# explosion/spacy-ray

Hardware: AMD Instinct MI355X
Metric: words/sec (whole node) en_core CNN tagger+parser+NER train (higher is better)
Workload: dtype bf16; 1 GPU; global_batch=1000015, seq_len=20, parallelism=dp1

## Files before the change

spacy_ray_amd/ops/api.py:

```python
from __future__ import annotations

import os
from typing import Optional

import torch

from . import torch_ref as ref

_HIP = None
_HIP_TRIED = False

FIXED_SCALE = 16777216.0


def deterministic() -> bool:
    return os.environ.get("SRX_DETERMINISTIC") == "1"


def hip_ext():
    global _HIP, _HIP_TRIED
    if not _HIP_TRIED:
        _HIP_TRIED = True
        try:
            from spacy_ray_amd import _srx_hip
# ... 717 lines not shown
    def forward(ctx, x, grad_buf):
        ctx.grad_buf = grad_buf
        ctx.dtype = x.dtype
        return x.new_zeros(())

    @staticmethod
    def backward(ctx, g):
        return ctx.grad_buf.to(ctx.dtype) * g, None


def inject_grad(x: torch.Tensor, grad_buf: torch.Tensor) -> torch.Tensor:
    return _InjectGrad.apply(x, grad_buf)


def parser_scatter_entries(entries, dPre32) -> None:
    if not entries:
        return
    hip = hip_ext()
    device = dPre32.device
    nF = entries[0][0].shape[1]
    HP = dPre32.shape[-1]
    feats_all = torch.cat([f for f, _ in entries], dim=0)
    dS_all = torch.cat([d for _, d in entries], dim=0).contiguous()
    SS = feats_all.shape[0]
    slot = torch.arange(nF, device=device)
    dest = (feats_all * nF + slot).reshape(-1).int()
    src = torch.arange(SS, device=device, dtype=torch.int32).repeat_interleave(nF)
    order = torch.argsort(dest)
    hip.seg_scatter_add(dest[order].contiguous(), src[order].contiguous(),
                        dS_all, dPre32.view(-1, HP))


class _MWELayer(torch.autograd.Function):

    @staticmethod
    def forward(ctx, X, weight, bias, g, b, starts, ends, dropmask, eps):
        Y, Mout, which, mu, rstd = hip_ext().mwe_layer_fwd(
            X.contiguous(), weight, bias, g, b, starts, ends, dropmask, eps
        )
        ctx.save_for_backward(X, weight, g, which, Mout, mu, rstd, starts, ends,
                              *( [dropmask] if dropmask is not None else [] ))
        ctx.has_mask = dropmask is not None
        return Y

    @staticmethod
    def backward(ctx, dY):
        if ctx.has_mask:
            X, weight, g, which, Mout, mu, rstd, starts, ends, dropmask = ctx.saved_tensors
        else:
            X, weight, g, which, Mout, mu, rstd, starts, ends = ctx.saved_tensors
            dropmask = None
        hip = hip_ext()
        dY = dY.contiguous()
        dPre, dX, dg32, db32, dbias32 = hip.mwe_bwd_fused(
            dY, dropmask, Mout, g, mu, rstd, which, weight, starts, ends)
        X3 = hip.seq2col_fwd(X, starts, ends)
        dW = mm_dw_chunked(dPre, X3)
        return (dX, dW, dbias32.to(dY.dtype), dg32.to(dY.dtype),
                db32.to(dY.dtype), None, None, None, None)


def mwe_layer(X, weight, bias, g, b, starts, ends, dropmask=None, eps: float = 1e-5):
    return _MWELayer.apply(X, weight, bias, g, b, starts, ends, dropmask, eps)


def mwe_layer_available(X: torch.Tensor, width: int, pieces: int) -> bool:
    return (
        X.is_cuda
        and X.dtype == torch.bfloat16
        and pieces == 3
        and width in (96, 128)
        and X.shape[0] % 64 == 0
        and hip_ext() is not None
    )


class _MixerLayer(torch.autograd.Function):

    @staticmethod
    def forward(ctx, E, weight, bias, g, b, dropmask, eps):
        E = E.contiguous()
        Y, Mout, which, mu, rstd = hip_ext().mixer_fwd(
            E, weight, bias, g, b, dropmask, eps)
        ctx.save_for_backward(E, weight, g, which, Mout, mu, rstd,
                              *([dropmask] if dropmask is not None else []))
        ctx.has_mask = dropmask is not None
        return Y

    @staticmethod
    def backward(ctx, dY):
        if ctx.has_mask:
            E, weight, g, which, Mout, mu, rstd, dropmask = ctx.saved_tensors
        else:
            E, weight, g, which, Mout, mu, rstd = ctx.saved_tensors
            dropmask = None
        dY = dY.contiguous()
        dPre, dE, dg32, db32, dbias32 = hip_ext().mixer_bwd_fused(
            dY, dropmask, Mout, g, mu, rstd, which, weight)
        dW = mm_dw_chunked(dPre, E)
        return (dE, dW, dbias32.to(dY.dtype), dg32.to(dY.dtype),
                db32.to(dY.dtype), None, None)


def mixer_layer(E, weight, bias, g, b, dropmask=None, eps: float = 1e-5):
    return _MixerLayer.apply(E, weight, bias, g, b, dropmask, eps)


def _mixer_composed() -> bool:
    mode = os.environ.get("SRX_MIXER", "")
    if mode not in ("", "composed"):
        raise ValueError(f"SRX_MIXER={mode!r}: expected 'composed' or unset")
    return mode == "composed"
# ... 271 lines not shown
```

spacy_ray_amd/ops/kernels/srx_ext.hip:

```cpp
#include <torch/extension.h>
#include <ATen/cuda/CUDAContext.h>

#include <mutex>
#include <unordered_map>
#include <utility>
#include <vector>

#include "srx_common.hip.h"
#include "srx_elementwise.hip.h"
#include "srx_embed_parser.hip.h"
#include "srx_softmax_reduce.hip.h"
#include "srx_mwe.hip.h"
#include "srx_mixer.hip.h"
#include "srx_staticvec.hip.h"
#include "srx_floret.hip.h"
#include "srx_vecloss.hip.h"
#include "srx_activations.hip.h"
#include "srx_attn.hip.h"

namespace {

constexpr int kBlock = 256;

inline int grid_for(long total, int per_thread = 1) {
  long blocks = (total + (long)kBlock * per_thread - 1) / ((long)kBlock * per_thread);
  return (int)std::min<long>(blocks, 16384);
}

inline void check_dev(const at::Tensor& t) {
  TORCH_CHECK(t.is_cuda(), "expected a GPU tensor");
  TORCH_CHECK(t.is_contiguous(), "expected contiguous");
}

#define DISPATCH_F(dtype, ...)                                        \
  if ((dtype) == at::kFloat) {                                        \
    using scalar_t = float;                                           \
    constexpr int kVec = 4;                                           \
    __VA_ARGS__;                                                      \
  } else if ((dtype) == at::kBFloat16) {                              \
    using scalar_t = bf16_t;                                          \
    constexpr int kVec = 8;                                           \
    __VA_ARGS__;                                                      \
  } else {                                                            \
    TORCH_CHECK(false, "unsupported dtype (need f32 or bf16)");       \
  }

at::Tensor seq2col_fwd(at::Tensor X, at::Tensor starts, at::Tensor ends) {
  check_dev(X);
  long nT = X.size(0);
  int W = (int)X.size(1);
  auto Y = at::empty({nT, 3L * W}, X.options());
  if (nT == 0) return Y;
  auto stream = at::cuda::getCurrentCUDAStream();
  DISPATCH_F(X.scalar_type(), {
    const int V = (W % kVec == 0) ? kVec : 1;
    long total = nT * 3L * (W / V);
    if (V == kVec)
      hipLaunchKernelGGL((seq2col_fwd_kernel<scalar_t, kVec>), dim3(grid_for(total)),
                         dim3(kBlock), 0, stream,
                         (const scalar_t*)X.data_ptr(), (scalar_t*)Y.data_ptr(),
                         starts.data_ptr<uint8_t>(), ends.data_ptr<uint8_t>(), nT, W);
    else
      hipLaunchKernelGGL((seq2col_fwd_kernel<scalar_t, 1>), dim3(grid_for(nT * 3L * W)),
                         dim3(kBlock), 0, stream,
                         (const scalar_t*)X.data_ptr(), (scalar_t*)Y.data_ptr(),
                         starts.data_ptr<uint8_t>(), ends.data_ptr<uint8_t>(), nT, W);
// ... 1058 lines not shown
  dim3 grid((unsigned)((T + C::MT - 1) / C::MT));
  hipLaunchKernelGGL((mwe_bwd_dx_kernel<W>), grid, dim3(C::NT), lds_bytes, stream,
                     (const bf16_t*)dPre.data_ptr(), (const bf16_t*)WT.data_ptr(),
                     starts.data_ptr<uint8_t>(), ends.data_ptr<uint8_t>(),
                     (const bf16_t*)dY.data_ptr(), (bf16_t*)dX.data_ptr(), T);
}

at::Tensor mwe_bwd_dx(at::Tensor dPre, at::Tensor weight, at::Tensor starts,
                      at::Tensor ends, at::Tensor dY) {
  check_dev(dPre);
  check_dev(dY);
  TORCH_CHECK(weight.is_cuda(), "expected a GPU tensor");
  TORCH_CHECK(dPre.scalar_type() == at::kBFloat16 &&
                  weight.scalar_type() == at::kBFloat16 &&
                  dY.scalar_type() == at::kBFloat16,
              "mwe_bwd_dx is bf16-only");
  TORCH_CHECK(dPre.dim() == 2 && dY.dim() == 2 && weight.dim() == 2,
              "mwe_bwd_dx expects 2-d tensors");
  long T = dY.size(0);
  int W = (int)dY.size(1);
  TORCH_CHECK(W == 96 || W == 128, "mwe_bwd_dx supports W in {96,128}");
  TORCH_CHECK(T % 64 == 0, "mwe_bwd_dx needs T % 64 == 0 (TokenBatch pads)");
  TORCH_CHECK(dPre.size(0) == T && dPre.size(1) == 3 * W, "dPre must be [T,3W]");
  TORCH_CHECK(weight.size(0) == 3 * W && weight.size(1) == 3 * W,
              "weight must be [3W,3W]");
  TORCH_CHECK(starts.numel() == T && ends.numel() == T,
              "starts/ends must have T entries");
  auto dX = at::empty_like(dY);
  if (T == 0) return dX;
  auto WT = weight.t().contiguous();
  auto stream = at::cuda::getCurrentCUDAStream();
  if (W == 96)
    launch_mwe_bwd_dx<96>(dPre, WT, starts, ends, dY, dX, T, stream);
  else
    launch_mwe_bwd_dx<128>(dPre, WT, starts, ends, dY, dX, T, stream);
  return dX;
}

at::Tensor mwe_fold_partials(at::Tensor part, int ncols, hipStream_t stream) {
  long n = part.size(0);
  const int R = 64;
  do {
    long nb = (n + R - 1) / R;
    auto out = at::empty({nb, (long)ncols}, part.options());
    hipLaunchKernelGGL(mwe_colsum_kernel, dim3((unsigned)nb, (ncols + 63) / 64),
                       dim3(64), 0, stream, part.data_ptr<float>(),
                       out.data_ptr<float>(), n, R, ncols);
    part = out;
    n = nb;
  } while (n > 1);
  return part.view({(long)ncols});
}

template <int W>
void launch_mwe_bwd_fused(const at::Tensor& dY,
                          const c10::optional<at::Tensor>& dropmask,
                          const at::Tensor& Mout, const at::Tensor& g,
                          const at::Tensor& mu, const at::Tensor& rstd,
                          const at::Tensor& which, const at::Tensor& WT,
                          const at::Tensor& starts, const at::Tensor& ends,
                          at::Tensor& dPre, at::Tensor& dX, at::Tensor& partials,
                          long T, hipStream_t stream) {
  using C = MweCfg<W, true>;
  size_t lds_bytes = (size_t)(C::A_ELEMS + C::B_ELEMS) * sizeof(bf16_t);
  static bool attr_set = false;
  if (!attr_set) {
    (void)hipFuncSetAttribute((const void*)mwe_bwd_fused_kernel<W>,
                              hipFuncAttributeMaxDynamicSharedMemorySize,
                              (int)lds_bytes);
    attr_set = true;
  }
  dim3 grid((unsigned)((T + C::MT - 1) / C::MT));
  hipLaunchKernelGGL((mwe_bwd_fused_kernel<W>), grid, dim3(C::NT), lds_bytes,
                     stream, (const bf16_t*)dY.data_ptr(),
                     dropmask ? (const bf16_t*)dropmask->data_ptr() : nullptr,
                     (const bf16_t*)Mout.data_ptr(), (const bf16_t*)g.data_ptr(),
                     mu.data_ptr<float>(), rstd.data_ptr<float>(),
                     which.data_ptr<uint8_t>(), (const bf16_t*)WT.data_ptr(),
                     starts.data_ptr<uint8_t>(), ends.data_ptr<uint8_t>(),
                     (bf16_t*)dPre.data_ptr(), (bf16_t*)dX.data_ptr(),
                     partials.data_ptr<float>(), T);
}

std::vector<at::Tensor> mwe_bwd_fused(at::Tensor dY,
                                      c10::optional<at::Tensor> dropmask,
                                      at::Tensor Mout, at::Tensor g,
                                      at::Tensor mu, at::Tensor rstd,
                                      at::Tensor which, at::Tensor weight,
                                      at::Tensor starts, at::Tensor ends) {
  check_dev(dY);
  check_dev(Mout);
  check_dev(g);
  check_dev(mu);
  check_dev(rstd);
  check_dev(which);
  check_dev(starts);
  check_dev(ends);
  TORCH_CHECK(weight.is_cuda(), "expected a GPU tensor");
  TORCH_CHECK(dY.scalar_type() == at::kBFloat16 &&
                  Mout.scalar_type() == at::kBFloat16 &&
                  g.scalar_type() == at::kBFloat16 &&
                  weight.scalar_type() == at::kBFloat16,
              "mwe_bwd_fused is bf16-only");
  TORCH_CHECK(dY.dim() == 2 && weight.dim() == 2,
              "mwe_bwd_fused expects 2-d tensors");
  long T = dY.size(0);
  int W = (int)dY.size(1);
  TORCH_CHECK(W == 96 || W == 128, "mwe_bwd_fused supports W in {96,128}");
  TORCH_CHECK(T % 64 == 0, "mwe_bwd_fused needs T % 64 == 0 (TokenBatch pads)");
  TORCH_CHECK(weight.size(0) == 3 * W && weight.size(1) == 3 * W,
              "weight must be [3W,3W]");
  TORCH_CHECK(starts.numel() == T && ends.numel() == T,
              "starts/ends must have T entries");
  TORCH_CHECK(starts.scalar_type() == at::kByte && ends.scalar_type() == at::kByte,
              "starts/ends must be uint8");
  TORCH_CHECK(Mout.dim() == 2 && Mout.size(0) == T && Mout.size(1) == W,
              "Mout must be [T,W]");
  TORCH_CHECK(which.scalar_type() == at::kByte && which.dim() == 2 &&
                  which.size(0) == T && which.size(1) == W,
              "which must be uint8 [T,W]");
  TORCH_CHECK(mu.scalar_type() == at::kFloat && rstd.scalar_type() == at::kFloat &&
                  mu.numel() == T && rstd.numel() == T,
              "mu/rstd must be fp32 with T entries");
  TORCH_CHECK(g.numel() == W, "g must have W entries");
  if (dropmask) {
    check_dev(*dropmask);
    TORCH_CHECK(dropmask->scalar_type() == at::kBFloat16 && dropmask->dim() == 2 &&
                    dropmask->size(0) == T && dropmask->size(1) == W,
                "dropmask must be bf16 [T,W]");
  }
  auto dPre = at::empty({T, 3L * W}, dY.options());
  auto dX = at::empty_like(dY);
  auto f32 = dY.options().dtype(at::kFloat);
  if (T == 0) {
    return {dPre, dX, at::zeros({W}, f32), at::zeros({W}, f32),
            at::zeros({3L * W}, f32)};
  }
  auto WT = weight.t().contiguous();
  auto stream = at::cuda::getCurrentCUDAStream();
  const int ncols = 5 * W;
  long n = (T + 127) / 128;
  auto part = at::empty({n, (long)ncols}, f32);
  if (W == 96)
    launch_mwe_bwd_fused<96>(dY, dropmask, Mout, g, mu, rstd, which, WT, starts,
                             ends, dPre, dX, part, T, stream);
  else
    launch_mwe_bwd_fused<128>(dY, dropmask, Mout, g, mu, rstd, which, WT, starts,
                              ends, dPre, dX, part, T, stream);
  auto sums = mwe_fold_partials(part, ncols, stream);
  return {dPre, dX, sums.narrow(0, 0, W), sums.narrow(0, W, W),
          sums.narrow(0, 2L * W, 3L * W)};
}

void mixer_check_shape(const char* name, long T, int W, int NS) {
  TORCH_CHECK(W == 96 || W == 128, name, " supports W in {96,128}");
  TORCH_CHECK(NS == 4 || NS == 5, name, " supports 4 or 5 input blocks of width W");
  TORCH_CHECK(T % 64 == 0, name, " needs T % 64 == 0 (TokenBatch pads)");
}

void mixer_check_mask(const c10::optional<at::Tensor>& dropmask, long T, int W) {
  if (!dropmask) return;
  check_dev(*dropmask);
  TORCH_CHECK(dropmask->scalar_type() == at::kBFloat16 && dropmask->dim() == 2 &&
                  dropmask->size(0) == T && dropmask->size(1) == W,
              "dropmask must be bf16 [T,W]");
}

template <int W, int NS>
void launch_mixer_fwd(const at::Tensor& E, const at::Tensor& Wm,
                      const at::Tensor& bias, const at::Tensor& g,
                      const at::Tensor& b,
                      const c10::optional<at::Tensor>& dropmask, at::Tensor& Y,
                      at::Tensor& Mout, at::Tensor& which, at::Tensor& mu,
                      at::Tensor& rstd, long T, double eps, hipStream_t stream) {
  using C = MixCfg<W, NS, false>;
  size_t lds_bytes = MixFwdLds<W, NS>::BYTES;
  static bool attr_set = false;
  if (!attr_set) {
    (void)hipFuncSetAttribute((const void*)mixer_fwd_kernel<W, NS>,
                              hipFuncAttributeMaxDynamicSharedMemorySize,
                              (int)lds_bytes);
    attr_set = true;
  }
  dim3 grid((unsigned)((T + C::MT - 1) / C::MT));
  hipLaunchKernelGGL((mixer_fwd_kernel<W, NS>), grid, dim3(C::NT), lds_bytes,
                     stream, (const bf16_t*)E.data_ptr(), (const bf16_t*)Wm.data_ptr(),
                     (const bf16_t*)bias.data_ptr(), (const bf16_t*)g.data_ptr(),
                     (const bf16_t*)b.data_ptr(),
                     dropmask ? (const bf16_t*)dropmask->data_ptr() : nullptr,
                     (bf16_t*)Y.data_ptr(), (bf16_t*)Mout.data_ptr(),
                     which.data_ptr<uint8_t>(), mu.data_ptr<float>(),
                     rstd.data_ptr<float>(), T, (float)eps);
}

std::vector<at::Tensor> mixer_fwd(at::Tensor E, at::Tensor Wm, at::Tensor bias,
                                  at::Tensor g, at::Tensor b,
                                  c10::optional<at::Tensor> dropmask, double eps) {
  check_dev(E);
  check_dev(Wm);
  check_dev(bias);
  check_dev(g);
  check_dev(b);
  TORCH_CHECK(E.scalar_type() == at::kBFloat16 &&
                  Wm.scalar_type() == at::kBFloat16 &&
// ... 442 lines not shown

std::vector<at::Tensor> srx_gpu_arceager(
    at::Tensor pre, at::Tensor off, at::Tensor lens, at::Tensor gh,
    at::Tensor gl, at::Tensor kids_off, at::Tensor kids, at::Tensor lowerB,
    at::Tensor upperW, at::Tensor upperB, int64_t total, int64_t n_labels,
    bool train, bool fuse_ce);
std::vector<at::Tensor> srx_gpu_biluo(
    at::Tensor pre, at::Tensor off, at::Tensor lens, at::Tensor gold,
    at::Tensor lowerB, at::Tensor upperW, at::Tensor upperB, int64_t total,
    int64_t n_types, bool train, bool fuse_ce);

PYBIND11_MODULE(TORCH_EXTENSION_NAME, m) {
  m.def("seq2col_fwd", &seq2col_fwd);
  m.def("seq2col_bwd", &seq2col_bwd, py::arg("dY"), py::arg("starts"),
        py::arg("ends"), py::arg("residual") = py::none());
  m.def("mwe_bwd_stage1", &mwe_bwd_stage1, py::arg("dY"), py::arg("dropmask"),
        py::arg("Mout"), py::arg("g"), py::arg("mu"), py::arg("rstd"),
        py::arg("which"), py::arg("deterministic") = false);
  m.def("maxout_fwd", &maxout_fwd);
  m.def("maxout_bwd", &maxout_bwd);
  m.def("layernorm_fwd", &layernorm_fwd);
  m.def("layernorm_bwd", &layernorm_bwd, py::arg("dY"), py::arg("X"),
        py::arg("g"), py::arg("mu"), py::arg("rstd"),
        py::arg("deterministic") = false);
  m.def("hashembed_fwd", &hashembed_fwd, py::arg("table"), py::arg("ids"),
        py::arg("seed"), py::arg("out") = py::none(), py::arg("col_off") = 0);
  m.def("hashembed_bwd", &hashembed_bwd);
  m.def("multi_hashembed_fwd", &multi_hashembed_fwd, py::arg("ids4"),
        py::arg("tables"), py::arg("seeds"), py::arg("X"), py::arg("col_off") = 0);
  m.def("hashembed_bwd_merged", &hashembed_bwd_merged, py::arg("order"),
        py::arg("rows"), py::arg("dY"), py::arg("dT32"));
  m.def("parser_step_fwd", &parser_step_fwd);
  m.def("parser_step_bwd", &parser_step_bwd);
  m.def("parser_step_bwd_into", &parser_step_bwd_into);
  m.def("action_select", &action_select);
  m.def("seg_scatter_add", &seg_scatter_add);
  m.def("adam_step", &adam_step);
  m.def("dropout_mask", &dropout_mask);
  m.def("act_fwd", &act_fwd);
  m.def("attn_softmax_fwd", &attn_softmax_fwd);
  m.def("attn_fused_fwd", &attn_fused_fwd);
  m.def("attn_fused_bwd", &attn_fused_bwd);
  m.def("attn_softmax_bwd", &attn_softmax_bwd);
  m.def("act_bwd", &act_bwd);
  m.def("softmax_ce", &softmax_ce);
  m.def("reduce_ragged", &reduce_ragged);
  m.def("reduce_ragged_bwd", &reduce_ragged_bwd);
  m.def("reduce_max_bwd", &reduce_max_bwd);
  m.def("mwe_layer_fwd", &mwe_layer_fwd);
  m.def("mwe_bwd_dx", &mwe_bwd_dx, py::arg("dPre"), py::arg("weight"),
        py::arg("starts"), py::arg("ends"), py::arg("dY"));
  m.def("mwe_bwd_fused", &mwe_bwd_fused, py::arg("dY"), py::arg("dropmask"),
        py::arg("Mout"), py::arg("g"), py::arg("mu"), py::arg("rstd"),
        py::arg("which"), py::arg("weight"), py::arg("starts"), py::arg("ends"));
  m.def("mixer_fwd", &mixer_fwd, py::arg("E"), py::arg("weight"), py::arg("bias"),
        py::arg("g"), py::arg("b"), py::arg("dropmask"), py::arg("eps"));
  m.def("mixer_bwd_fused", &mixer_bwd_fused, py::arg("dY"), py::arg("dropmask"),
        py::arg("Mout"), py::arg("g"), py::arg("mu"), py::arg("rstd"),
        py::arg("which"), py::arg("weight"));
  m.def("static_vectors_fwd", &static_vectors_fwd, py::arg("table"),
        py::arg("rows"), py::arg("W"), py::arg("Y"), py::arg("col_off") = 0);
  m.def("static_vectors_bwd_dw", &static_vectors_bwd_dw, py::arg("table"),
        py::arg("rows"), py::arg("dX"), py::arg("col_off"), py::arg("nO"),
        py::arg("max_groups") = 0, py::arg("nM") = 0);
  m.def("floret_words_mean", &floret_words_mean, py::arg("table"),
        py::arg("offsets"), py::arg("idx"), py::arg("out"));
  m.def("vectors_loss", &vectors_loss, py::arg("pred"), py::arg("table"),
        py::arg("rows"), py::arg("row_loss"), py::arg("dpred"), py::arg("l2"),
        py::arg("scale"));
  m.def("fused_step", &fusedstep::fused_step);
  m.def("fused_entries_take", &fusedstep::fused_entries_take);
  m.def("transition_ce", &transition_ce, py::arg("scores"), py::arg("gold"),
        py::arg("valid"), py::arg("deterministic") = false);
  m.attr("FIXED_SCALE") = 16777216.0;
  m.def("dpre_scatter", &dpre_scatter);
  m.def("dpre_scatter_docmajor", &dpre_scatter_docmajor);
  m.def("run_transition_loop", &srx_run_transition_loop,
        py::call_guard<py::gil_scoped_release>());
  m.def("gpu_arceager", &srx_gpu_arceager, py::arg("pre"), py::arg("off"),
        py::arg("lens"), py::arg("gh"), py::arg("gl"), py::arg("kids_off"),
        py::arg("kids"), py::arg("lowerB"), py::arg("upperW"),
        py::arg("upperB"), py::arg("total"), py::arg("n_labels"),
        py::arg("train"), py::arg("fuse_ce") = false);
  m.def("gpu_biluo", &srx_gpu_biluo, py::arg("pre"), py::arg("off"),
        py::arg("lens"), py::arg("gold"), py::arg("lowerB"), py::arg("upperW"),
        py::arg("upperB"), py::arg("total"), py::arg("n_types"),
        py::arg("train"), py::arg("fuse_ce") = false);
  m.attr("GPU_STATE_MAXLEN") = 128;
}
```

spacy_ray_amd/ops/kernels/srx_mwe.hip.h:

```cpp
#pragma once
#include "srx_common.hip.h"

typedef __attribute__((__vector_size__(8 * sizeof(short)))) short srx_bf16x8;
typedef __attribute__((__vector_size__(16 * sizeof(float)))) float srx_f32x16;

template <int W_, bool BWD_>
struct MweCfg {
  static constexpr int W = W_;
  static constexpr bool BWD = BWD_;
  static constexpr int NW = W / 32;
  static constexpr int MT = 128;
  static constexpr int NT = 64 * 2 * NW;
  static constexpr int KA = BWD ? 3 * W : W;
  static constexpr int AP = KA + 8;
  static constexpr int KC = BWD ? 96 : 32;
  static constexpr int BP = KC + 8;
  static constexpr int NBR = BWD ? W : 3 * W;
  static constexpr int LDB = 3 * W;
  static constexpr int NP = BWD ? 1 : 3;
  static constexpr int CPS = KA / KC;
  static constexpr int NC = 3 * CPS;
  static constexpr int PF = NBR * (KC / 8) / NT;
  static constexpr int A_ROWS = MT + 2;
  static constexpr int A_ELEMS = A_ROWS * AP;
// ... 392 lines not shown
  const long nwaves = ((long)gridDim.x * blockDim.x) / SRX_WAVE;
  const int ncols = (W + SRX_WAVE - 1) / SRX_WAVE;
  float dg_loc[4], db_loc[4], dbias_loc[4 * 3];
  for (int c = 0; c < ncols; c++) { dg_loc[c] = 0.f; db_loc[c] = 0.f; }
  for (int k = 0; k < ncols * 3; k++) dbias_loc[k] = 0.f;
  for (long n = wave; n < N; n += nwaves) {
    const T* dyrow = dY + n * (long)W;
    const T* mrow = Mout + n * (long)W;
    const T* maskrow = dropmask ? dropmask + n * (long)W : nullptr;
    float m = mu[n], r = rstd[n];
    float s1 = 0.f, s2 = 0.f;
    float dl[4], xh[4];
    for (int c = 0; c < ncols; c++) {
      int w = lane + c * SRX_WAVE;
      if (w >= W) { dl[c] = 0.f; xh[c] = 0.f; continue; }
      float d = Elem<T>::ld(dyrow + w);
      if (maskrow) d *= Elem<T>::ld(maskrow + w);
      float xhat = (Elem<T>::ld(mrow + w) - m) * r;
      float dxhat = d * Elem<T>::ld(g + w);
      dl[c] = d;
      xh[c] = xhat;
      s1 += dxhat;
      s2 += dxhat * xhat;
      dg_loc[c] += d * xhat;
      db_loc[c] += d;
    }
    s1 = wave_reduce_sum(s1) / W;
    s2 = wave_reduce_sum(s2) / W;
    T* out = dPre + n * (long)(3 * W);
    const uint8_t* wrow = which + n * (long)W;
    for (int c = 0; c < ncols; c++) {
      int w = lane + c * SRX_WAVE;
      if (w >= W) continue;
      float dxhat = dl[c] * Elem<T>::ld(g + w);
      float dM = r * (dxhat - s1 - xh[c] * s2);
      int p = wrow[w];
      for (int q = 0; q < 3; q++)
        Elem<T>::st(out + q * W + w, q == p ? dM : 0.f);
      dbias_loc[c * 3 + p] += dM;
    }
  }
  for (int c = 0; c < ncols; c++) {
    int w = lane + c * SRX_WAVE;
    if (w >= W) continue;
    if (dg_loc[c] != 0.f) srx_atomic_add<DET>(dg32, w, dg_loc[c]);
    if (db_loc[c] != 0.f) srx_atomic_add<DET>(db32, w, db_loc[c]);
    for (int q = 0; q < 3; q++)
      if (dbias_loc[c * 3 + q] != 0.f)
        srx_atomic_add<DET>(dbias32, (long)q * W + w, dbias_loc[c * 3 + q]);
  }
}


template <int W, int NT, int AP, int HALO>
__device__ __forceinline__ void mwe_stage1_tile(
    const bf16_t* __restrict__ dY, const bf16_t* __restrict__ dropmask,
    const bf16_t* __restrict__ Mout, const bf16_t* __restrict__ g,
    const float* __restrict__ mu, const float* __restrict__ rstd,
    const uint8_t* __restrict__ which, long T, long t0, int tid, bf16_t* ldsA,
    float (&dg_out)[8], float (&db_out)[8], float (&dbias_out)[3][8]) {
  constexpr int MT = 128, A_ROWS = MT + 2 * HALO;
  constexpr int Q = W / 8;
  constexpr int RG = NT / 16;
  constexpr int NPASS = (A_ROWS + RG - 1) / RG;
  const int q = tid & 15, rg = tid >> 4;
  const bool qv = q < Q;
  float gv[8];
#pragma unroll
  for (int j = 0; j < 8; j++) gv[j] = 0.f;
  if (qv) ElemV<bf16_t, 8>::ld(g + q * 8, gv);

  srx_u32x4_t rdy[NPASS], rmk[NPASS], rmo[NPASS];
  uint2 rwh[NPASS];
  float rmu[NPASS], rrs[NPASS];
#pragma unroll
  for (int ps = 0; ps < NPASS; ps++) {
    const int i = ps * RG + rg;
    const long t = t0 - HALO + i;
    rdy[ps] = srx_u32x4_t{0u, 0u, 0u, 0u};
    rmk[ps] = srx_u32x4_t{0u, 0u, 0u, 0u};
    rmo[ps] = srx_u32x4_t{0u, 0u, 0u, 0u};
    rwh[ps] = make_uint2(0u, 0u);
    rmu[ps] = 0.f;
    rrs[ps] = 0.f;
    if (qv && i < A_ROWS && t >= 0 && t < T) {
      rdy[ps] = *(const srx_u32x4_t*)(dY + t * W + q * 8);
      if (dropmask) rmk[ps] = *(const srx_u32x4_t*)(dropmask + t * W + q * 8);
      rmo[ps] = *(const srx_u32x4_t*)(Mout + t * W + q * 8);
      rwh[ps] = *(const uint2*)(which + t * W + q * 8);
      rmu[ps] = mu[t];
      rrs[ps] = rstd[t];
    }
  }

  float dg_loc[8], db_loc[8], dbias_loc[3][8];
#pragma unroll
  for (int j = 0; j < 8; j++) {
    dg_loc[j] = 0.f;
    db_loc[j] = 0.f;
    dbias_loc[0][j] = dbias_loc[1][j] = dbias_loc[2][j] = 0.f;
  }

#pragma unroll
  for (int ps = 0; ps < NPASS; ps++) {
    const int i = ps * RG + rg;
    const long t = t0 - HALO + i;
    const bool live = qv && i < A_ROWS && t >= 0 && t < T;
    const bool own = live && i >= HALO && i < MT + HALO;
    const float m = rmu[ps], r = rrs[ps];
    float d[8], xh[8], dxh[8];
    float s1 = 0.f, s2 = 0.f;
#pragma unroll
    for (int j = 0; j < 8; j++) {
      const int sh = 16 * (j & 1);
      d[j] = bf2f((bf16_t)((rdy[ps][j >> 1] >> sh) & 0xffffu));
      if (dropmask) d[j] *= bf2f((bf16_t)((rmk[ps][j >> 1] >> sh) & 0xffffu));
      xh[j] = (bf2f((bf16_t)((rmo[ps][j >> 1] >> sh) & 0xffffu)) - m) * r;
      dxh[j] = d[j] * gv[j];
      s1 += dxh[j];
      s2 += dxh[j] * xh[j];
    }
#pragma unroll
    for (int off = 1; off < 16; off <<= 1) {
      s1 += __shfl_xor(s1, off, SRX_WAVE);
      s2 += __shfl_xor(s2, off, SRX_WAVE);
    }
    s1 = s1 / W;
    s2 = s2 / W;
    uint32_t hb[8], wh[8];
#pragma unroll
    for (int j = 0; j < 8; j++) {
      const float dM = r * (dxh[j] - s1 - xh[j] * s2);
      wh[j] = ((j < 4 ? rwh[ps].x : rwh[ps].y) >> (8 * (j & 3))) & 0xffu;
      hb[j] = live ? (uint32_t)f2bf(dM) : 0u;
      if (own) {
        dg_loc[j] = fmaf(d[j], xh[j], dg_loc[j]);
        db_loc[j] += d[j];
#pragma unroll
        for (int p = 0; p < 3; p++) dbias_loc[p][j] += (wh[j] == (uint32_t)p) ? dM : 0.f;
      }
    }
    if (qv && i < A_ROWS) {
#pragma unroll
      for (int p = 0; p < 3; p++) {
        srx_u32x4_t o;
#pragma unroll
        for (int k = 0; k < 4; k++)
          o[k] = (wh[2 * k] == (uint32_t)p ? hb[2 * k] : 0u) |
                 ((wh[2 * k + 1] == (uint32_t)p ? hb[2 * k + 1] : 0u) << 16);
        *(srx_u32x4_t*)(ldsA + i * AP + p * W + q * 8) = o;
      }
    }
  }
#pragma unroll
  for (int j = 0; j < 8; j++) {
    dg_out[j] = dg_loc[j];
    db_out[j] = db_loc[j];
#pragma unroll
    for (int p = 0; p < 3; p++) dbias_out[p][j] = dbias_loc[p][j];
  }
}

template <int W>
__device__ __forceinline__ void mwe_colsums_park(float (&dg_loc)[8],
                                                 float (&db_loc)[8],
                                                 float (&dbias_loc)[3][8],
                                                 float* ldsC, int tid) {
  const int lane = tid % SRX_WAVE, wave = tid / SRX_WAVE;
  const int q = tid & 15;
  const bool qv = q < W / 8;
#pragma unroll
  for (int j = 0; j < 8; j++) {
#pragma unroll
    for (int off = 16; off < SRX_WAVE; off <<= 1) {
      dg_loc[j] += __shfl_xor(dg_loc[j], off, SRX_WAVE);
      db_loc[j] += __shfl_xor(db_loc[j], off, SRX_WAVE);
#pragma unroll
      for (int p = 0; p < 3; p++)
        dbias_loc[p][j] += __shfl_xor(dbias_loc[p][j], off, SRX_WAVE);
    }
  }
  if (lane < 16 && qv) {
    float* row = ldsC + wave * (5 * W) + q * 8;
    ElemV<float, 4>::st(row, dg_loc);
    ElemV<float, 4>::st(row + 4, dg_loc + 4);
    ElemV<float, 4>::st(row + W, db_loc);
    ElemV<float, 4>::st(row + W + 4, db_loc + 4);
#pragma unroll
    for (int p = 0; p < 3; p++) {
      ElemV<float, 4>::st(row + (2 + p) * W, dbias_loc[p]);
      ElemV<float, 4>::st(row + (2 + p) * W + 4, dbias_loc[p] + 4);
    }
  }
}

template <int W, int NT>
__device__ __forceinline__ void mwe_colsums_out(const float* ldsC,
                                                float* __restrict__ out, int tid) {
  for (int c = tid; c < 5 * W; c += NT) {
    float s = 0.f;
#pragma unroll
    for (int wv = 0; wv < NT / SRX_WAVE; wv++) s += ldsC[wv * (5 * W) + c];
    out[c] = s;
  }
}

template <int W>
__global__ __launch_bounds__(4 * W) void mwe_bwd_fused_kernel(
    const bf16_t* __restrict__ dY,
    const bf16_t* __restrict__ dropmask,
    const bf16_t* __restrict__ Mout,
    const bf16_t* __restrict__ g,
    const float* __restrict__ mu,
    const float* __restrict__ rstd,
    const uint8_t* __restrict__ which,
    const bf16_t* __restrict__ WT,
    const uint8_t* __restrict__ is_start,
    const uint8_t* __restrict__ is_end,
    bf16_t* __restrict__ dPre,
    bf16_t* __restrict__ dX,
    float* __restrict__ partials,
    long T) {
  using C = MweCfg<W, true>;
  constexpr int NW = C::NW, MT = C::MT, NT = C::NT, AP = C::AP;
  constexpr int Q = W / 8;
  constexpr int NWAVE = NT / SRX_WAVE;
  constexpr int OP = W + 4;
  static_assert(MT * OP * 4 <= C::A_ELEMS * 2, "output tile");
  static_assert(NWAVE * 5 * W * 4 <= C::B_ELEMS * 2, "column-sum partials");
  extern __shared__ __attribute__((aligned(16))) bf16_t lds[];
  bf16_t* ldsA = lds;
  bf16_t* ldsB = lds + C::A_ELEMS;
  float* ldsO = (float*)lds;
  float* ldsC = (float*)ldsB;

  const int tid = threadIdx.x;
  const int lane = tid % SRX_WAVE;
  const int wave = tid / SRX_WAVE;
  const int mh = wave / NW, w = wave % NW;
  const long t0 = (long)blockIdx.x * MT;

  srx_u32x4_t pf[C::PF];
  mwe_b_fetch<C>(WT, 0, tid, pf);

  float dg_loc[8], db_loc[8], dbias_loc[3][8];
  mwe_stage1_tile<W, NT, AP, 1>(dY, dropmask, Mout, g, mu, rstd, which, T, t0,
                                tid, ldsA, dg_loc, db_loc, dbias_loc);

  int zmask[2];
  mwe_section_masks<C>(is_start, is_end, T, t0, mh, lane, zmask);
  mwe_b_store<C>(ldsB, tid, pf);
  __syncthreads();

  for (int id = tid; id < MT * (3 * Q); id += NT) {
    const int r = id / (3 * Q), c = id % (3 * Q);
    if (t0 + r < T)
      *(srx_u32x4_t*)(dPre + (t0 + r) * (3 * W) + c * 8) =
          *(const srx_u32x4_t*)(ldsA + (r + 1) * AP + c * 8);
  }

  srx_f32x16 acc[1][2];
  mwe_chunk_loop<C>(WT, ldsA, ldsB, zmask, pf, acc);

  mwe_colsums_park<W>(dg_loc, db_loc, dbias_loc, ldsC, tid);

  const int col = 32 * w + (lane & 31);
#pragma unroll
  for (int mi = 0; mi < 2; mi++)
#pragma unroll
    for (int rr = 0; rr < 16; rr++) {
      const int r = 64 * mh + 32 * mi + (rr & 3) + 8 * (rr >> 2) + 4 * (lane >> 5);
      ldsO[r * OP + col] = acc[0][mi][rr];
    }
  __syncthreads();
  for (int id = tid; id < MT * Q; id += NT) {
    const int r = id / Q, qq = id % Q;
    if (t0 + r < T) {
      float v[8], d[8];
      ElemV<bf16_t, 8>::ld(dY + (t0 + r) * W + qq * 8, d);
      const float4 lo = *(const float4*)(ldsO + r * OP + qq * 8);
      const float4 hi = *(const float4*)(ldsO + r * OP + qq * 8 + 4);
      v[0] = lo.x + d[0]; v[1] = lo.y + d[1]; v[2] = lo.z + d[2]; v[3] = lo.w + d[3];
      v[4] = hi.x + d[4]; v[5] = hi.y + d[5]; v[6] = hi.z + d[6]; v[7] = hi.w + d[7];
      ElemV<bf16_t, 8>::st(dX + (t0 + r) * W + qq * 8, v);
    }
  }
  mwe_colsums_out<W, NT>(ldsC, partials + (long)blockIdx.x * (5 * W), tid);
}

__global__ void mwe_colsum_kernel(const float* __restrict__ in,
                                  float* __restrict__ out, long n, int R,
                                  int ncols) {
  const int c = blockIdx.y * blockDim.x + threadIdx.x;
  if (c >= ncols) return;
  const long r0 = (long)blockIdx.x * R;
  const long r1 = r0 + R < n ? r0 + R : n;
  double s = 0.0;
  for (long r = r0; r < r1; r++) s += (double)in[r * ncols + c];
  out[(long)blockIdx.x * ncols + c] = (float)s;
}
```

Measured before the change: 28.02 million words/s.

## Compute maxout weight gradient from compact dM with a fused persistent kernel

For width 96, the fused backward kernel now writes a compact [T,W] dM instead of the [T,3W] piece-scattered dPre. A new persistent MFMA kernel rebuilds the per-piece masks from `which` and the seq2col windows from X in LDS on the fly, then accumulates the 288x288 weight gradient per workgroup. A deterministic fp64 reduction over workgroups produces the final bf16 dW. This removes the 3x-wide dPre write, the materialized seq2col X3 tensor and the chunked matmul, at the cost of a complex custom kernel, redundant masked MFMAs per piece, and an extra [G,288,288] fp32 workspace.

```diff
diff --git a/spacy_ray_amd/ops/api.py b/spacy_ray_amd/ops/api.py
--- a/spacy_ray_amd/ops/api.py
+++ b/spacy_ray_amd/ops/api.py
@@ -793,12 +793,30 @@
             dropmask = None
         hip = hip_ext()
         dY = dY.contiguous()
-        dPre, dX, dg32, db32, dbias32 = hip.mwe_bwd_fused(
-            dY, dropmask, Mout, g, mu, rstd, which, weight, starts, ends)
-        X3 = hip.seq2col_fwd(X, starts, ends)
-        dW = mm_dw_chunked(dPre, X3)
+        if mwe_dw_available(X.shape[1]):
+            dM, dX, dg32, db32, dbias32 = hip.mwe_bwd_fused(
+                dY, dropmask, Mout, g, mu, rstd, which, weight, starts, ends,
+                compact=True)
+            dW = hip.mwe_bwd_dw(dM, which, X.contiguous(), starts, ends)
+        else:
+            dPre, dX, dg32, db32, dbias32 = hip.mwe_bwd_fused(
+                dY, dropmask, Mout, g, mu, rstd, which, weight, starts, ends)
+            X3 = hip.seq2col_fwd(X, starts, ends)
+            dW = mm_dw_chunked(dPre, X3)
         return (dX, dW, dbias32.to(dY.dtype), dg32.to(dY.dtype),
                 db32.to(dY.dtype), None, None, None, None)
+
+
+def _mwe_dw_composed() -> bool:
+    mode = os.environ.get("SRX_MWE_DW", "")
+    if mode not in ("", "composed"):
+        raise ValueError(f"SRX_MWE_DW={mode!r}: expected 'composed' or unset")
+    return mode == "composed"
+
+
+def mwe_dw_available(width: int) -> bool:
+    composed = _mwe_dw_composed()
+    return (not composed) and width == 96
 
 
 def mwe_layer(X, weight, bias, g, b, starts, ends, dropmask=None, eps: float = 1e-5):
diff --git a/spacy_ray_amd/ops/kernels/srx_ext.hip b/spacy_ray_amd/ops/kernels/srx_ext.hip
--- a/spacy_ray_amd/ops/kernels/srx_ext.hip
+++ b/spacy_ray_amd/ops/kernels/srx_ext.hip
@@ -12,6 +12,7 @@
 #include "srx_softmax_reduce.hip.h"
 #include "srx_mwe.hip.h"
 #include "srx_mixer.hip.h"
+#include "srx_mwe_dw.hip.h"
 #include "srx_staticvec.hip.h"
 #include "srx_floret.hip.h"
 #include "srx_vecloss.hip.h"
@@ -1176,7 +1177,7 @@
   return part.view({(long)ncols});
 }
 
-template <int W>
+template <int W, bool COMPACT>
 void launch_mwe_bwd_fused(const at::Tensor& dY,
                           const c10::optional<at::Tensor>& dropmask,
                           const at::Tensor& Mout, const at::Tensor& g,
@@ -1189,13 +1190,13 @@
   size_t lds_bytes = (size_t)(C::A_ELEMS + C::B_ELEMS) * sizeof(bf16_t);
   static bool attr_set = false;
   if (!attr_set) {
-    (void)hipFuncSetAttribute((const void*)mwe_bwd_fused_kernel<W>,
+    (void)hipFuncSetAttribute((const void*)mwe_bwd_fused_kernel<W, COMPACT>,
                               hipFuncAttributeMaxDynamicSharedMemorySize,
                               (int)lds_bytes);
     attr_set = true;
   }
   dim3 grid((unsigned)((T + C::MT - 1) / C::MT));
-  hipLaunchKernelGGL((mwe_bwd_fused_kernel<W>), grid, dim3(C::NT), lds_bytes,
+  hipLaunchKernelGGL((mwe_bwd_fused_kernel<W, COMPACT>), grid, dim3(C::NT), lds_bytes,
                      stream, (const bf16_t*)dY.data_ptr(),
                      dropmask ? (const bf16_t*)dropmask->data_ptr() : nullptr,
                      (const bf16_t*)Mout.data_ptr(), (const bf16_t*)g.data_ptr(),
@@ -1211,7 +1212,8 @@
                                       at::Tensor Mout, at::Tensor g,
                                       at::Tensor mu, at::Tensor rstd,
                                       at::Tensor which, at::Tensor weight,
-                                      at::Tensor starts, at::Tensor ends) {
+                                      at::Tensor starts, at::Tensor ends,
+                                      bool compact) {
   check_dev(dY);
   check_dev(Mout);
   check_dev(g);
@@ -1253,7 +1255,7 @@
                     dropmask->size(0) == T && dropmask->size(1) == W,
                 "dropmask must be bf16 [T,W]");
   }
-  auto dPre = at::empty({T, 3L * W}, dY.options());
+  auto dPre = at::empty({T, (compact ? 1L : 3L) * W}, dY.options());
   auto dX = at::empty_like(dY);
   auto f32 = dY.options().dtype(at::kFloat);
   if (T == 0) {
@@ -1265,15 +1267,79 @@
   const int ncols = 5 * W;
   long n = (T + 127) / 128;
   auto part = at::empty({n, (long)ncols}, f32);
-  if (W == 96)
-    launch_mwe_bwd_fused<96>(dY, dropmask, Mout, g, mu, rstd, which, WT, starts,
-                             ends, dPre, dX, part, T, stream);
+  if (W == 96 && compact)
+    launch_mwe_bwd_fused<96, true>(dY, dropmask, Mout, g, mu, rstd, which, WT,
+                                   starts, ends, dPre, dX, part, T, stream);
+  else if (W == 96)
+    launch_mwe_bwd_fused<96, false>(dY, dropmask, Mout, g, mu, rstd, which, WT,
+                                    starts, ends, dPre, dX, part, T, stream);
+  else if (compact)
+    launch_mwe_bwd_fused<128, true>(dY, dropmask, Mout, g, mu, rstd, which, WT,
+                                    starts, ends, dPre, dX, part, T, stream);
   else
-    launch_mwe_bwd_fused<128>(dY, dropmask, Mout, g, mu, rstd, which, WT, starts,
-                              ends, dPre, dX, part, T, stream);
+    launch_mwe_bwd_fused<128, false>(dY, dropmask, Mout, g, mu, rstd, which, WT,
+                                     starts, ends, dPre, dX, part, T, stream);
   auto sums = mwe_fold_partials(part, ncols, stream);
   return {dPre, dX, sums.narrow(0, 0, W), sums.narrow(0, W, W),
           sums.narrow(0, 2L * W, 3L * W)};
+}
+
+at::Tensor mwe_bwd_dw(at::Tensor dM, at::Tensor which, at::Tensor X,
+                      at::Tensor starts, at::Tensor ends, int64_t max_groups) {
+  check_dev(dM);
+  check_dev(which);
+  check_dev(X);
+  check_dev(starts);
+  check_dev(ends);
+  TORCH_CHECK(which.device() == dM.device() && X.device() == dM.device() &&
+                  starts.device() == dM.device() && ends.device() == dM.device(),
+              "mwe_bwd_dw: all tensors must be on one device");
+  TORCH_CHECK(dM.scalar_type() == at::kBFloat16 && X.scalar_type() == at::kBFloat16,
+              "mwe_bwd_dw is bf16-only");
+  TORCH_CHECK(dM.dim() == 2 && X.dim() == 2 && which.dim() == 2,
+              "mwe_bwd_dw expects 2-d tensors");
+  TORCH_CHECK(dM.is_contiguous() && X.is_contiguous() && which.is_contiguous() &&
+                  starts.is_contiguous() && ends.is_contiguous(),
+              "mwe_bwd_dw expects contiguous tensors");
+  const long T = dM.size(0);
+  const int W = (int)dM.size(1);
+  TORCH_CHECK(W == 96, "mwe_bwd_dw supports W = 96");
+  TORCH_CHECK(T % 64 == 0, "mwe_bwd_dw needs T % 64 == 0 (TokenBatch pads)");
+  TORCH_CHECK(X.size(0) == T && X.size(1) == W, "X must be [T,W]");
+  TORCH_CHECK(which.scalar_type() == at::kByte && which.size(0) == T &&
+                  which.size(1) == W,
+              "which must be uint8 [T,W]");
+  TORCH_CHECK(starts.scalar_type() == at::kByte && ends.scalar_type() == at::kByte,
+              "starts/ends must be uint8");
+  TORCH_CHECK(starts.dim() == 1 && ends.dim() == 1 && starts.numel() == T &&
+                  ends.numel() == T,
+              "starts/ends must have T entries");
+  if (T == 0) return at::zeros({3L * W, 3L * W}, dM.options());
+  using C = MweDwCfg<96>;
+  const long ntiles = (T + C::MT - 1) / C::MT;
+  long G = std::min<long>(ntiles,
+                          at::cuda::getCurrentDeviceProperties()->multiProcessorCount);
+  if (max_groups > 0) G = std::min<long>(G, max_groups);
+  const int n = 9 * W * W;
+  auto ws = at::empty({G, 3L * W, 3L * W}, dM.options().dtype(at::kFloat));
+  auto dW = at::empty({3L * W, 3L * W}, dM.options());
+  auto stream = at::cuda::getCurrentCUDAStream();
+  static bool attr_set = false;
+  if (!attr_set) {
+    (void)hipFuncSetAttribute((const void*)mwe_bwd_dw_kernel<96>,
+                              hipFuncAttributeMaxDynamicSharedMemorySize,
+                              (int)C::LDS_BYTES);
+    attr_set = true;
+  }
+  hipLaunchKernelGGL((mwe_bwd_dw_kernel<96>), dim3((unsigned)G), dim3(C::NT),
+                     (size_t)C::LDS_BYTES, stream, (const bf16_t*)dM.data_ptr(),
+                     which.data_ptr<uint8_t>(), (const bf16_t*)X.data_ptr(),
+                     starts.data_ptr<uint8_t>(), ends.data_ptr<uint8_t>(),
+                     ws.data_ptr<float>(), T, (int)ntiles);
+  hipLaunchKernelGGL(mwe_dw_reduce_kernel, dim3((n + kBlock - 1) / kBlock),
+                     dim3(kBlock), 0, stream, ws.data_ptr<float>(),
+                     (bf16_t*)dW.data_ptr(), (int)G, n);
+  return dW;
 }
 
 void mixer_check_shape(const char* name, long T, int W, int NS) {
@@ -1822,7 +1888,10 @@
         py::arg("starts"), py::arg("ends"), py::arg("dY"));
   m.def("mwe_bwd_fused", &mwe_bwd_fused, py::arg("dY"), py::arg("dropmask"),
         py::arg("Mout"), py::arg("g"), py::arg("mu"), py::arg("rstd"),
-        py::arg("which"), py::arg("weight"), py::arg("starts"), py::arg("ends"));
+        py::arg("which"), py::arg("weight"), py::arg("starts"), py::arg("ends"),
+        py::arg("compact") = false);
+  m.def("mwe_bwd_dw", &mwe_bwd_dw, py::arg("dM"), py::arg("which"), py::arg("X"),
+        py::arg("starts"), py::arg("ends"), py::arg("max_groups") = 0);
   m.def("mixer_fwd", &mixer_fwd, py::arg("E"), py::arg("weight"), py::arg("bias"),
         py::arg("g"), py::arg("b"), py::arg("dropmask"), py::arg("eps"));
   m.def("mixer_bwd_fused", &mixer_bwd_fused, py::arg("dY"), py::arg("dropmask"),
diff --git a/spacy_ray_amd/ops/kernels/srx_mwe.hip.h b/spacy_ray_amd/ops/kernels/srx_mwe.hip.h
--- a/spacy_ray_amd/ops/kernels/srx_mwe.hip.h
+++ b/spacy_ray_amd/ops/kernels/srx_mwe.hip.h
@@ -468,13 +468,14 @@
 }
 
 
-template <int W, int NT, int AP, int HALO>
+template <int W, int NT, int AP, int HALO, bool COMPACT = false>
 __device__ __forceinline__ void mwe_stage1_tile(
     const bf16_t* __restrict__ dY, const bf16_t* __restrict__ dropmask,
     const bf16_t* __restrict__ Mout, const bf16_t* __restrict__ g,
     const float* __restrict__ mu, const float* __restrict__ rstd,
     const uint8_t* __restrict__ which, long T, long t0, int tid, bf16_t* ldsA,
-    float (&dg_out)[8], float (&db_out)[8], float (&dbias_out)[3][8]) {
+    float (&dg_out)[8], float (&db_out)[8], float (&dbias_out)[3][8],
+    bf16_t* __restrict__ dMout = nullptr) {
   constexpr int MT = 128, A_ROWS = MT + 2 * HALO;
   constexpr int Q = W / 8;
   constexpr int RG = NT / 16;
@@ -556,6 +557,12 @@
         for (int p = 0; p < 3; p++) dbias_loc[p][j] += (wh[j] == (uint32_t)p) ? dM : 0.f;
       }
     }
+    if (COMPACT && own) {
+      srx_u32x4_t o;
+#pragma unroll
+      for (int k = 0; k < 4; k++) o[k] = hb[2 * k] | (hb[2 * k + 1] << 16);
+      *(srx_u32x4_t*)(dMout + t * W + q * 8) = o;
+    }
     if (qv && i < A_ROWS) {
 #pragma unroll
       for (int p = 0; p < 3; p++) {
@@ -621,7 +628,7 @@
   }
 }
 
-template <int W>
+template <int W, bool COMPACT = false>
 __global__ __launch_bounds__(4 * W) void mwe_bwd_fused_kernel(
     const bf16_t* __restrict__ dY,
     const bf16_t* __restrict__ dropmask,
@@ -660,15 +667,16 @@
   mwe_b_fetch<C>(WT, 0, tid, pf);
 
   float dg_loc[8], db_loc[8], dbias_loc[3][8];
-  mwe_stage1_tile<W, NT, AP, 1>(dY, dropmask, Mout, g, mu, rstd, which, T, t0,
-                                tid, ldsA, dg_loc, db_loc, dbias_loc);
+  mwe_stage1_tile<W, NT, AP, 1, COMPACT>(dY, dropmask, Mout, g, mu, rstd, which,
+                                         T, t0, tid, ldsA, dg_loc, db_loc,
+                                         dbias_loc, dPre);
 
   int zmask[2];
   mwe_section_masks<C>(is_start, is_end, T, t0, mh, lane, zmask);
   mwe_b_store<C>(ldsB, tid, pf);
   __syncthreads();
 
-  for (int id = tid; id < MT * (3 * Q); id += NT) {
+  for (int id = tid; !COMPACT && id < MT * (3 * Q); id += NT) {
     const int r = id / (3 * Q), c = id % (3 * Q);
     if (t0 + r < T)
       *(srx_u32x4_t*)(dPre + (t0 + r) * (3 * W) + c * 8) =
diff --git a/spacy_ray_amd/ops/kernels/srx_mwe_dw.hip.h b/spacy_ray_amd/ops/kernels/srx_mwe_dw.hip.h
--- /dev/null
+++ b/spacy_ray_amd/ops/kernels/srx_mwe_dw.hip.h
@@ -0,0 +1,218 @@
+#pragma once
+#include "srx_common.hip.h"
+#include "srx_mwe.hip.h"
+#include "srx_staticvec.hip.h"
+
+typedef __attribute__((__vector_size__(4 * sizeof(float)))) float srx_f32x4;
+
+template <int W_>
+struct MweDwCfg {
+  static constexpr int W = W_;
+  static constexpr int MT = 128;
+  static constexpr int NWAVE = W / 8;
+  static constexpr int NT = 64 * NWAVE;
+  static constexpr int CT = W / 16;
+  static constexpr int JH = NWAVE / CT;
+  static constexpr int NJ = CT / JH;
+  static constexpr int TP = MT + 8;
+  static constexpr int NIMG = 5;
+  static constexpr int RP = NIMG * TP;
+  static constexpr int LDS_BYTES = W * RP * 2;
+  static_assert(W == 96, "mwe_bwd_dw_kernel: 288 x 288 accumulators, 12 waves");
+  static_assert(NWAVE == CT * JH && CT == NJ * JH, "wave decomposition");
+};
+
+struct MweDwPrefetch {
+  srx_u32x4_t da, db;
+  srx_u32x4_t xa, xb;
+  srx_u32x4_t xh;
+  uint2 wa, wb;
+  uint32_t bnd;
+};
+
+template <int W>
+__device__ __forceinline__ void mwe_dw_fetch(
+    const bf16_t* __restrict__ dM, const uint8_t* __restrict__ which,
+    const bf16_t* __restrict__ X, const uint8_t* __restrict__ is_start,
+    const uint8_t* __restrict__ is_end, long T, long t0, int q, int lane,
+    MweDwPrefetch& pf) {
+  const srx_u32x4_t zero = {0u, 0u, 0u, 0u};
+  const long ta = t0 + 2 * lane;
+  pf.da = pf.db = pf.xa = pf.xb = pf.xh = zero;
+  pf.wa = pf.wb = make_uint2(0u, 0u);
+  pf.bnd = 0u;
+  if (ta < T) {
+    const long o = ta * W + q * 8;
+    pf.da = *(const srx_u32x4_t*)(dM + o);
+    pf.db = *(const srx_u32x4_t*)(dM + o + W);
+    pf.xa = *(const srx_u32x4_t*)(X + o);
+    pf.xb = *(const srx_u32x4_t*)(X + o + W);
+    pf.wa = *(const uint2*)(which + o);
+    pf.wb = *(const uint2*)(which + o + W);
+    pf.bnd = (is_start[ta] ? 1u : 0u) | (is_start[ta + 1] ? 2u : 0u) |
+             (is_end[ta] ? 4u : 0u) | (is_end[ta + 1] ? 8u : 0u);
+  }
+  if (lane == 0 && t0 > 0)
+    pf.xh = *(const srx_u32x4_t*)(X + (t0 - 1) * W + q * 8);
+  if (lane == 63 && t0 + 128 < T)
+    pf.xh = *(const srx_u32x4_t*)(X + (t0 + 128) * W + q * 8);
+}
+
+__device__ __forceinline__ srx_u32x4_t mwe_dw_shfl_up1(const srx_u32x4_t& v) {
+  srx_u32x4_t r;
+#pragma unroll
+  for (int k = 0; k < 4; k++) r[k] = __shfl_up(v[k], 1, SRX_WAVE);
+  return r;
+}
+
+__device__ __forceinline__ srx_u32x4_t mwe_dw_shfl_down1(const srx_u32x4_t& v) {
+  srx_u32x4_t r;
+#pragma unroll
+  for (int k = 0; k < 4; k++) r[k] = __shfl_down(v[k], 1, SRX_WAVE);
+  return r;
+}
+
+__device__ __forceinline__ int mwe_dw_dword(int m, int q, int e, int l0) {
+  return (q * 8 + e) * 340 + m * 68 + (e < 4 ? l0 : (l0 ^ 4));
+}
+
+__device__ __forceinline__ void mwe_dw_store_tr(bf16_t* lds, int m, int q, int l0,
+                                                const srx_u32x4_t& v0,
+                                                const srx_u32x4_t& v1,
+                                                uint32_t mask) {
+#pragma unroll
+  for (int e = 0; e < 8; e++) {
+    const uint32_t lo = sv_half(v0, e), hi = sv_half(v1, e);
+    ((uint32_t*)lds)[mwe_dw_dword(m, q, e, l0)] = (lo | (hi << 16)) & mask;
+  }
+}
+
+template <int W>
+__device__ __forceinline__ void mwe_dw_stage(const MweDwPrefetch& pf, int q,
+                                             int lane, bf16_t* lds) {
+  static_assert(MweDwCfg<W>::RP == 2 * 340, "mwe_dw_dword");
+  const int l0 = lane ^ ((q & 1) << 2);
+  mwe_dw_store_tr(lds, 0, q, l0, pf.da, pf.db, 0xffffffffu);
+#pragma unroll
+  for (int e = 0; e < 8; e++) {
+    const uint32_t ba = ((e < 4 ? pf.wa.x : pf.wa.y) >> (8 * (e & 3))) & 0xffu;
+    const uint32_t bb = ((e < 4 ? pf.wb.x : pf.wb.y) >> (8 * (e & 3))) & 0xffu;
+    ((uint32_t*)lds)[mwe_dw_dword(1, q, e, l0)] = (1u << ba) | ((1u << bb) << 16);
+  }
+  srx_u32x4_t prevb = mwe_dw_shfl_up1(pf.xb);
+  srx_u32x4_t nexta = mwe_dw_shfl_down1(pf.xa);
+  if (lane == 0) prevb = pf.xh;
+  if (lane == 63) nexta = pf.xh;
+  const uint32_t m0 = ((pf.bnd & 1u) ? 0u : 0x0000ffffu) |
+                      ((pf.bnd & 2u) ? 0u : 0xffff0000u);
+  const uint32_t m2 = ((pf.bnd & 4u) ? 0u : 0x0000ffffu) |
+                      ((pf.bnd & 8u) ? 0u : 0xffff0000u);
+  mwe_dw_store_tr(lds, 2, q, l0, prevb, pf.xa, m0);
+  mwe_dw_store_tr(lds, 3, q, l0, pf.xa, pf.xb, 0xffffffffu);
+  mwe_dw_store_tr(lds, 4, q, l0, pf.xb, nexta, m2);
+}
+
+template <int W>
+__global__ __launch_bounds__(8 * W) void mwe_bwd_dw_kernel(
+    const bf16_t* __restrict__ dM,
+    const uint8_t* __restrict__ which,
+    const bf16_t* __restrict__ X,
+    const uint8_t* __restrict__ is_start,
+    const uint8_t* __restrict__ is_end,
+    float* __restrict__ ws,
+    long T, int ntiles) {
+  using C = MweDwCfg<W>;
+  extern __shared__ __attribute__((aligned(16))) bf16_t lds[];
+
+  const int tid = threadIdx.x;
+  const int lane = tid % SRX_WAVE;
+  const int wave = __builtin_amdgcn_readfirstlane(tid / SRX_WAVE);
+  const int ct = wave % C::CT, jh = wave / C::CT;
+  const int r = lane & 15, g = lane >> 4;
+
+  srx_f32x4 acc[3][C::NJ][3];
+#pragma unroll
+  for (int p = 0; p < 3; p++)
+#pragma unroll
+    for (int jj = 0; jj < C::NJ; jj++)
+#pragma unroll
+      for (int s = 0; s < 3; s++)
+#pragma unroll
+        for (int k = 0; k < 4; k++) acc[p][jj][s][k] = 0.f;
+
+  const int coff = (8 * g) ^ (((r + 4) & 8) ? 8 : 0);
+  const bf16_t* arow = lds + (16 * ct + r) * C::RP + coff;
+  const bf16_t* crow = arow + C::TP;
+  const bf16_t* xrow = lds + (16 * C::NJ * jh + r) * C::RP + 2 * C::TP + coff;
+
+  MweDwPrefetch pf;
+  int tile = blockIdx.x;
+  if (tile < ntiles)
+    mwe_dw_fetch<W>(dM, which, X, is_start, is_end, T, (long)tile * C::MT, wave,
+                    lane, pf);
+  for (; tile < ntiles; tile += gridDim.x) {
+    mwe_dw_stage<W>(pf, wave, lane, lds);
+    __syncthreads();
+    const int next = tile + gridDim.x;
+    if (next < ntiles)
+      mwe_dw_fetch<W>(dM, which, X, is_start, is_end, T, (long)next * C::MT, wave,
+                      lane, pf);
+
+#pragma unroll 1
+    for (int ks = 0; ks < C::MT / 32; ks++) {
+      const int off = 32 * ks;
+      const srx_u32x4_t dmf = *(const srx_u32x4_t*)(arow + off);
+      const srx_u32x4_t cdf = *(const srx_u32x4_t*)(crow + off);
+      srx_bf16x8 afrag[3];
+#pragma unroll
+      for (int p = 0; p < 3; p++) {
+        srx_u32x4_t a;
+#pragma unroll
+        for (int k = 0; k < 4; k++) {
+          const uint32_t m = (cdf[k] >> p) & 0x00010001u;
+          a[k] = dmf[k] & ((m << 16) - m);
+        }
+        afrag[p] = (srx_bf16x8)a;
+      }
+#pragma unroll
+      for (int jj = 0; jj < C::NJ; jj++) {
+#pragma unroll
+        for (int s = 0; s < 3; s++) {
+          const srx_bf16x8 bfrag =
+              *(const srx_bf16x8*)(xrow + s * C::TP + jj * 16 * C::RP + off);
+#pragma unroll
+          for (int p = 0; p < 3; p++)
+            acc[p][jj][s] = __builtin_amdgcn_mfma_f32_16x16x32_bf16(
+                afrag[p], bfrag, acc[p][jj][s], 0, 0, 0);
+        }
+      }
+    }
+    __syncthreads();
+  }
+
+  const int el = __builtin_amdgcn_mbcnt_hi(~0u, __builtin_amdgcn_mbcnt_lo(~0u, 0u));
+  const int er = el & 15, eg = el >> 4;
+  float* out = ws + (long)blockIdx.x * (3 * W) * (3 * W);
+#pragma unroll
+  for (int p = 0; p < 3; p++)
+#pragma unroll
+    for (int jj = 0; jj < C::NJ; jj++)
+#pragma unroll
+      for (int s = 0; s < 3; s++)
+#pragma unroll
+        for (int k = 0; k < 4; k++) {
+          const int row = p * W + 16 * ct + 4 * eg + k;
+          const int col = s * W + 16 * (C::NJ * jh + jj) + er;
+          out[(long)row * (3 * W) + col] = acc[p][jj][s][k];
+        }
+}
+
+__global__ void mwe_dw_reduce_kernel(const float* __restrict__ ws,
+                                     bf16_t* __restrict__ dW, int G, int n) {
+  const int i = blockIdx.x * blockDim.x + threadIdx.x;
+  if (i >= n) return;
+  double s = 0.0;
+#pragma unroll 8
+  for (int gi = 0; gi < G; gi++) s += (double)ws[(long)gi * n + i];
+  dW[i] = f2bf((float)s);
+}
```

New measurement: 29.18 million words/s (median of 6 runs). 4.1% higher.
